# Chemical118/TREW

Hardware: AMD Instinct MI355X
Metric: Gbases/s scanned (short 5 32, 150 bp reads) (higher is better)
Workload: dtype u32

## Files before the change

### trew_amd/csrc/kernels/prefilter.inc

```


#ifdef TREW_MARK_READ_SETUP
#define TREW_SETUP_MARK(n) asm volatile("; MARK " #n)
#else
#define TREW_SETUP_MARK(n)
#endif

__device__ __forceinline__ u32 xor_and(u32 x, u32 y, u32 m) { return __builtin_amdgcn_bitop3_b32(x, y, m, 0x28); }

__device__ __forceinline__ u64 all_k_mask(int kmin, int kmax) {
    if (kmax < kmin) return 0;
    u64 hi = kmax >= 64 ? ~0ull : ((1ull << kmax) - 1ull);
    u64 lo = (1ull << (kmin - 1)) - 1ull;
    return hi & ~lo;
}

template <int NW, int WS>
__device__ __forceinline__ u32 shr_word(const u32 (&x)[NW], int j, u32 bs) {
    const u32 lo = (j + WS < NW) ? x[j + WS < NW ? j + WS : 0] : 0u;
    const u32 hi = (j + WS + 1 < NW) ? x[j + WS + 1 < NW ? j + WS + 1 : 0] : 0u;
    return alignbit(hi, lo, bs);
}

template <int NW, int WS, int NWW>
// ... 346 lines not shown
}
__device__ __forceinline__ u32 halves_note(u32 acc, u32 x, u32 t) { return __builtin_amdgcn_bitop3_b32(acc, x, t, 0x40); }
struct Thr8 {
    int4 a, b;
};
__device__ __forceinline__ Thr8 load_thr8(const int4 *p) {
    typedef int v8i __attribute__((ext_vector_type(8)));
    typedef const __attribute__((address_space(4))) v8i *cptr;
    const v8i v = *(cptr) (unsigned long long) p;
    Thr8 o;
    o.a = make_int4(v[0], v[1], v[2], v[3]);
    o.b = make_int4(v[4], v[5], v[6], v[7]);
    return o;
}
__device__ __forceinline__ int4 load_thr4(const int4 *p) {
    typedef int v4i __attribute__((ext_vector_type(4)));
    typedef const __attribute__((address_space(4))) v4i *cptr;
    const v4i v = *(cptr) (unsigned long long) p;
    return make_int4(v.x, v.y, v.z, v.w);
}

__device__ __forceinline__ const int4 *joint_thresholds(const int2 *thr_tab) { return (const int4 *) (thr_tab + kThrRows * kThrRow); }

__device__ __forceinline__ void filter_halves_uni(const HalvesP &A, const HalvesP &Bh, int L, int klo, int khi, const int4 *__restrict__ thr_row,
                                                  const u32 *wm_tab, bool &passA, bool &passB) {
    u32 accA = 0xffffffffu, accB = 0xffffffffu;
    int k = klo;
    const int4 *tp = thr_row + (klo - 1);
    {
        int b = L - 64;
        b = b > khi ? khi : b;
        auto probe = [&](u32 bs, const int4 t) __attribute__((always_inline)) {
            u32 xA, tA, xB, tB;
            halves_signs(A.P1[0] ^ alignbit(A.P1[1], A.P1[0], bs), A.P2[0] ^ alignbit(A.P2[1], A.P2[0], bs), A.P1[1] ^ alignbit(A.P1[2], A.P1[1], bs),
                         A.P2[1] ^ alignbit(A.P2[2], A.P2[1], bs), t.x, t.y, t.z, xA, tA);
            halves_signs(Bh.P1[0] ^ alignbit(Bh.P1[1], Bh.P1[0], bs), Bh.P2[0] ^ alignbit(Bh.P2[1], Bh.P2[0], bs), Bh.P1[1] ^ alignbit(Bh.P1[2], Bh.P1[1], bs),
                         Bh.P2[1] ^ alignbit(Bh.P2[2], Bh.P2[1], bs), t.x, t.y, t.z, xB, tB);
            accA = halves_note(accA, xA, tA);
            accB = halves_note(accB, xB, tB);
        };
        for (; k + 1 <= b; k += 2, tp += 2) {
            const Thr8 t8 = load_thr8(tp);
            probe((u32) k, t8.a);
            probe((u32) k + 1u, t8.b);
        }
        if (k <= b) {
// ... 51 lines not shown
    V[0] &= alignbit(V[1], V[0], 1u);
    V[1] &= alignbit(V[2], V[1], 1u);
    V[2] &= V[2] >> 1;
}
template <int N>
__device__ __forceinline__ int drain_signs(const u32 (&F1)[N], const u32 (&F2)[N], const int4 th) {
    u32 a = (u32) th.x, b = (u32) th.x, c = (u32) th.y;
#pragma unroll
    for (int j = 0; j < N; j++) {
        a = bcnt_acc(F1[j], a);
        b = bcnt_acc(F2[j], b);
        c = bcnt_acc(F1[j] & F2[j], c);
    }
    const u32 p = a - c, q = b - c;
    const u32 t = a + q + (u32) th.z;
    return (int) __builtin_amdgcn_bitop3_b32(__builtin_amdgcn_bitop3_b32(p, q, c, 0x80), t, t, 0x30);
}
template <int N>
__device__ __forceinline__ bool drain_pass8(const u32 (&F1)[N], const u32 (&F2)[N], const u32 (&F3)[N], const u32 (&V)[N], u32 count, int ithr) {
    const u32 m8 = max_bucket8<N>(F1, F2, F3, V, count);
    return (int) m8 >= ithr;
}

__device__ __forceinline__ bool drain_uni_applies(const DevParams &P, u32 UL, int gmax_run) {
    const int n_halves = P.mode == TREW_MODE_PAIR ? 4 : (P.mode == TREW_MODE_SHORT ? 2 : 0);
    if (n_halves == 0) return false;
    for (int slot = n_halves; slot < mode_slots(P.mode); slot++)
        if (get_segment(P.mode, slot, UL, UL, P.min_mer, P.max_mer, P.slice_len).valid) return false;
    const Segment first = get_segment(P.mode, 0, UL, UL, P.min_mer, P.max_mer, P.slice_len);
    for (int p = 0; p < n_halves; p += 2) {
        const Segment a = get_segment(P.mode, p, UL, UL, P.min_mer, P.max_mer, P.slice_len);
        const Segment b = get_segment(P.mode, p + 1, UL, UL, P.min_mer, P.max_mer, P.slice_len);
        const int la = (int) a.len, lb = (int) b.len, lmin = la < lb ? la : lb, lmax = la < lb ? lb : la;
        const int khi = a.kmax < gmax_run ? a.kmax : gmax_run;
        if (!(a.valid && b.valid && a.kmin == b.kmin && a.kmax == b.kmax && lmax <= 95 && lmax - lmin <= 1 && a.kmin >= 1 && khi <= lmin)) return false;
        if (a.kmin != first.kmin || a.kmax != first.kmax) return false;
    }
    return true;
}

__device__ __forceinline__ u64 drain_probe3(const DrainHalf &h, u32 bs, u64 flag, const int4 *cnt_thr) {
    const u32 cnt = bcnt_acc(h.V[2], bcnt_acc(h.V[1], __popc(h.V[0])));
    const int4 th = cnt_thr[cnt];
    u32 F1[3], F2[3];
#pragma unroll
    for (int j = 0; j < 3; j++) {
        F1[j] = xor_and(h.P1[j], alignbit(j < 2 ? h.P1[j < 2 ? j + 1 : 0] : 0u, h.P1[j], bs), h.V[j]);
        F2[j] = xor_and(h.P2[j], alignbit(j < 2 ? h.P2[j < 2 ? j + 1 : 0] : 0u, h.P2[j], bs), h.V[j]);
    }
    const u64 p4 = __ballot(drain_signs<3>(F1, F2, th) >= 0);
    u64 p8 = 0;
    if (p4 & ~flag) {
        u32 F3[3];
#pragma unroll
        for (int j = 0; j < 3; j++) F3[j] = h.P3[j] ^ alignbit(j < 2 ? h.P3[j < 2 ? j + 1 : 0] : 0u, h.P3[j], bs);
        p8 = __ballot(drain_pass8<3>(F1, F2, F3, h.V, cnt, th.w));
    }
    return p8;
}
__device__ __forceinline__ u64 drain_probe2(const DrainHalf &h, u64 Q1, u64 Q2, u64 V, int s, int k, u64 flag, const int4 *cnt_thr) {
    const u32 v0 = (u32) V, v1 = (u32) (V >> 32);
    const u32 cnt = bcnt_acc(v1, __popc(v0));
    const int4 th = cnt_thr[cnt];
    const u32 sh = (u32) (k - s);
    const u64 S1 = Q1 >> sh, S2 = Q2 >> sh;
    const u32 F1[2] = {xor_and(h.P1[0], (u32) S1, v0), xor_and(h.P1[1], (u32) (S1 >> 32), v1)};
    const u32 F2[2] = {xor_and(h.P2[0], (u32) S2, v0), xor_and(h.P2[1], (u32) (S2 >> 32), v1)};
    const u64 p4 = __ballot(drain_signs<2>(F1, F2, th) >= 0);
    u64 p8 = 0;
    if (p4 & ~flag) {
        const u64 S3 = container64(h.P3, s) >> sh;
        const u32 F3[2] = {h.P3[0] ^ (u32) S3, h.P3[1] ^ (u32) (S3 >> 32)};
        const u32 Vw[2] = {v0, v1};
        p8 = __ballot(drain_pass8<2>(F1, F2, F3, Vw, cnt, th.w));
    }
    return p8;
}

__device__ __forceinline__ bool filter_deferred_uni(const DevParams &P, const DevBatch &B, u64 unit, bool active, int gmax_run,
                                                    const int4 *cnt_thr) {
    const u32 UL = B.uniform_length;
    ReadRef rd[2];
    unit_reads(P, B, unit, active, rd);
    const u64 actm = __ballot(active);
    u64 flag = 0;
    const int n_halves = P.mode == TREW_MODE_PAIR ? 4 : 2;
    for (int p = 0; p < n_halves && flag != actm; p += 2) {
        const Segment sA = get_segment(P.mode, p, UL, UL, P.min_mer, P.max_mer, P.slice_len);
        const Segment sB = get_segment(P.mode, p + 1, UL, UL, P.min_mer, P.max_mer, P.slice_len);
        const int LA = rfl_i((int) sA.len), LB = rfl_i((int) sB.len), Lmax = LA < LB ? LB : LA;
        const int klo = rfl_i(sA.kmin > P.min_mer ? sA.kmin : P.min_mer), khi = rfl_i(sA.kmax < gmax_run ? sA.kmax : gmax_run);
        DrainHalf A, Bh;
        {
            u32 lo[3], hi[3], nm[3];
            load_planes<3>(sA.mate ? rd[1] : rd[0], sA.start, lo, hi, nm);
            drain_half_init(lo, hi, nm, LA, active, A);
            load_planes<3>(sB.mate ? rd[1] : rd[0], sB.start, lo, hi, nm);
            drain_half_init(lo, hi, nm, LB, active, Bh);
        }
        for (int t = 1; t < klo; t++) {
            drain_v_step3(A.V);
            drain_v_step3(Bh.V);
        }
        int k = klo;
        for (const int b = khi < Lmax - 64 ? khi : Lmax - 64; k <= b && flag != actm; k++) {
            flag |= drain_probe3(A, (u32) k, flag, cnt_thr);
            flag |= drain_probe3(Bh, (u32) k, flag, cnt_thr);
            drain_v_step3(A.V);
            drain_v_step3(Bh.V);
        }
        if (k <= khi && flag != actm) {
            const int oA = LA > 63 ? LA - 63 : 0, oB = LB > 63 ? LB - 63 : 0;
            const u64 QA1 = container64(A.P1, oA), QA2 = container64(A.P2, oA), QB1 = container64(Bh.P1, oB), QB2 = container64(Bh.P2, oB);
            u64 VA = ((u64) A.V[1] << 32) | A.V[0], VB = ((u64) Bh.V[1] << 32) | Bh.V[0];
            for (; k <= khi && flag != actm; k++) {
                flag |= drain_probe2(A, QA1, QA2, VA, oA, k, flag, cnt_thr);
                flag |= drain_probe2(Bh, QB1, QB2, VB, oB, k, flag, cnt_thr);
                VA &= VA >> 1;
                VB &= VB >> 1;
            }
        }
    }
    return (flag >> lane_id()) & 1ull;
}

__device__ __forceinline__ bool filter_deferred_half(const DevParams &P, const DevBatch &B, u64 unit, u32 half, bool active, int gmax_run,
                                                     const int4 *cnt_thr) {
    const u32 UL = B.uniform_length;
    ReadRef rd[2];
    unit_reads(P, B, unit, active, rd);
    Segment sg = get_segment(P.mode, 0, UL, UL, P.min_mer, P.max_mer, P.slice_len);
    int Lmax = (int) sg.len;
    const int n_halves = P.mode == TREW_MODE_PAIR ? 4 : 2;
    for (int slot = 1; slot < n_halves; slot++) {
        const Segment o = get_segment(P.mode, slot, UL, UL, P.min_mer, P.max_mer, P.slice_len);
        Lmax = (int) o.len > Lmax ? (int) o.len : Lmax;
        if (half == (u32) slot) {
            sg.mate = o.mate;
            sg.start = o.start;
            sg.len = o.len;
        }
    }
    Lmax = rfl_i(Lmax);
    const int L = (int) sg.len;
    const int klo = rfl_i(sg.kmin > P.min_mer ? sg.kmin : P.min_mer), khi = rfl_i(sg.kmax < gmax_run ? sg.kmax : gmax_run);
    DrainHalf h;
    {
        u32 lo[3], hi[3], nm[3];
        load_planes<3>(sg.mate ? rd[1] : rd[0], sg.start, lo, hi, nm);
        drain_half_init(lo, hi, nm, L, active, h);
    }
    for (int t = 1; t < klo; t++) drain_v_step3(h.V);
    const u64 actm = __ballot(active);
    u64 flag = 0;
    int k = klo;
    for (const int b = khi < Lmax - 64 ? khi : Lmax - 64; k <= b && flag != actm; k++) {
        flag |= drain_probe3(h, (u32) k, flag, cnt_thr);
        drain_v_step3(h.V);
    }
    if (k <= khi && flag != actm) {
        const int o = L > 63 ? L - 63 : 0;
        const u64 Q1 = container64(h.P1, o), Q2 = container64(h.P2, o);
        u64 V = ((u64) h.V[1] << 32) | h.V[0];
        for (; k <= khi && flag != actm; k++) {
            flag |= drain_probe2(h, Q1, Q2, V, o, k, flag, cnt_thr);
            V &= V >> 1;
        }
    }
    return (flag >> lane_id()) & 1ull;
}

constexpr u32 kFilterThreads = TREW_FILTER_THREADS;
// ... 26 lines not shown
            __syncthreads();
            const u32 fb = flush_base;
            for (u32 i = threadIdx.x; i < n; i += blockDim.x) {
                if (fb + i < wl_cap)
                    wl[fb + i] = stage[i];
                else
                    atomicAdd(&diag[kDiagWorklistDrop], 1u);
            }
            __syncthreads();
            if (threadIdx.x == 0) stage_n = 0;
        }
        __syncthreads();
    };
    auto append = [&](bool flag, u32 unit) __attribute__((always_inline)) {
        wave_append(&stage_n, flag, [&](u32 at) __attribute__((always_inline)) { stage[at] = unit; });
        __syncthreads();
        const bool full = stage_n > kStage - kFilterThreads;
        defer_seen = defer_n;
        if constexpr (NW == 3) half_seen = half_n;
        __syncthreads();
        if (full) flush();
    };
    const int nslots = mode_slots(P.mode);
    const int gmax_run = (P.flags & TREW_FLAG_DEBUG_NO_KLOOP) ? P.min_mer - 1 : P.max_mer;
    auto general = [&](u64 unit, bool active) __attribute__((always_inline)) -> u64 {
        ReadRef rd[2];
        unit_reads(P, B, unit, active, rd);
        u64 any = 0;
#pragma unroll
        for (int slot = 0; slot < kMaxSlots; slot++) {
            if (slot < nslots) {
                u64 mask = 0;
                Segment sg = get_segment(P.mode, slot, rd[0].len, rd[1].len, P.min_mer, P.max_mer, P.slice_len);
                const bool ok = active && sg.valid && sg.len <= (u32) (32 * NW - 1);
                if (__any(ok)) {
                    u32 lo[NW], hi[NW], nm[NW];
                    const ReadRef &r = sg.mate ? rd[1] : rd[0];
                    if (ok) {
                        load_planes<NW>(r, sg.start, lo, hi, nm);
                    } else {
#pragma unroll
                        for (int j = 0; j < NW; j++) {
                            lo[j] = hi[j] = 0;
                            nm[j] = 0xffffffffu;
                        }
                    }
                    u64 m;
// ... 1 lines not shown
                        m = all_k_mask(sg.kmin, sg.kmax);
                    else
                        m = filter_segment<NW>(lo, hi, nm, ok ? (int) sg.len : 0, sg.kmin, sg.kmax, P.min_mer, gmax_run, max_seg, P.lowf);
                    mask = ok ? m : 0ull;
                }
                if (active && sg.valid && sg.len > (u32) (32 * NW - 1)) mask = all_k_mask(sg.kmin, sg.kmax);
                any |= mask;
                if (dbg_masks && active && slot < dbg_slots) dbg_masks[unit * (u64) dbg_slots + slot] = mask;
            }
        }
        return any;
    };

    __shared__ u32 defer[kDefer];
    __shared__ unsigned char defer_kind[kDefer];
    constexpr u32 kHalfDefer = NW == 3 ? kDefer : 1;
    __shared__ u32 hdefer[kHalfDefer];
    __shared__ unsigned char hdefer_kind[kHalfDefer];
    __shared__ u32 wm_tab[34];
    if (threadIdx.x < 34) wm_tab[threadIdx.x] = threadIdx.x < 32 ? 0xffffffffu >> threadIdx.x : 0u;
    __shared__ int4 cnt_thr[kCntThr];
    for (u32 i = threadIdx.x; i < (u32) kCntThr; i += blockDim.x) cnt_thr[i] = count_thresholds((int) i, P.lowf);
    const u32 UL = B.uniform_length;
    const bool uni = NW <= 5 && UL != 0 && thr_tab != nullptr && P.mode != TREW_MODE_LONG && !(P.flags & TREW_FLAG_NO_FILTER);
    const bool uni_drain = NW == 3 && uni && !dbg_masks && !(P.flags & TREW_FLAG_DEBUG_NO_UNI_DRAIN) && drain_uni_applies(P, UL, gmax_run);
    if (threadIdx.x == 0) defer_n = 0;
    if constexpr (NW == 3) {
        if (threadIdx.x == 0) half_n = 0;
    }
    __syncthreads();
    __shared__ u32 next_chunk[2];
    constexpr u32 kChunkShards = 8;
    const u32 my_shard = blockIdx.x & (kChunkShards - 1u);
    auto shard_ctr = [&](u32 sh) __attribute__((always_inline)) { return wl_count + 32u + 32u * sh + kChunkCounterWord; };
    u64 chunk = blockIdx.x;
    u32 round = 0;
    for (;;) {
        const bool more = chunk * kFilterThreads < B.n_units;
        if (more) {
            const u64 unit = chunk * kFilterThreads + threadIdx.x;
            const bool active = unit < B.n_units;
            u32 nxt = 0;
            if (threadIdx.x == 0) nxt = gridDim.x + kChunkShards * atomicAdd(shard_ctr(my_shard), 1u) + my_shard;
            u64 any = 0;
            bool dfr = active, dfr_n = false;
            bool dfr_half = false;
            u32 hsel = 0;
            if constexpr (NW <= 5) {
                if (uni) {
                    TREW_SETUP_MARK(read_setup);
                    ReadRef rd[2];
                    unit_reads(P, B, unit, active, rd);
                    dfr = false;
                    int slot0 = 0;
                    if constexpr (NW == 3) {
                        const int n_halves = P.mode == TREW_MODE_PAIR ? 4 : (P.mode == TREW_MODE_SHORT ? 2 : 0);
                        u32 nneed = 0;
                        for (; slot0 + 1 < n_halves && !dbg_masks && !(P.flags & TREW_FLAG_DEBUG_NO_JOINT); slot0 += 2) {
                            const Segment sA = get_segment(P.mode, slot0, UL, UL, P.min_mer, P.max_mer, P.slice_len);
                            const Segment sB = get_segment(P.mode, slot0 + 1, UL, UL, P.min_mer, P.max_mer, P.slice_len);
                            const int L = rfl_i((int) sA.len);
                            const int klo = rfl_i(sA.kmin > P.min_mer ? sA.kmin : P.min_mer), khi = rfl_i(sA.kmax < gmax_run ? sA.kmax : gmax_run);
                            const bool uneq = sB.len == sA.len + 1u;
                            if (!(sA.valid && sB.valid && (sA.len == sB.len || uneq) && sA.len <= 95u && sA.kmin == sB.kmin && sA.kmax == sB.kmax &&
                                  klo >= L + 1 - kUniSubsetMax && khi <= L - 32 && klo <= 31))
                                break;
                            HalvesP hp, hq;
                            u32 np, nq;
                            u32 slot_p = (u32) slot0, slot_q = (u32) slot0 + 1u;
                            const bool a_left = sA.start == 0u;
                            const u32 h = rfl(a_left ? sB.start : sA.start), len_l = rfl(a_left ? sA.len : sB.len), len_r = rfl(a_left ? sB.len : sA.len);
                            const bool one_load = UL <= 159u && sA.mate == sB.mate && (a_left ? sA.start : sB.start) == 0u && (h >> 5) == 2u && h + len_r <= UL;
                            if (one_load) {
                                TREW_SETUP_MARK(one_load);
                                ReadPlanes5 r;
                                load_read5(sA.mate ? rd[1] : rd[0], r);
                                np = read5_left_has_n(r.nm, (int) len_l);
                                nq = read5_right_has_n(r.nm, (int) h, (int) len_r);
                                if (!a_left) slot_p = (u32) slot0 + 1u, slot_q = (u32) slot0;
#ifndef TREW_AB_NO_READ_PREFIX
                                halves_prefix_read5(r, h & 31u, hp, hq);
#else
                                u32 loq[3], hiq[3];
                                read5_from64(r.lo, h & 31u, loq);
                                read5_from64(r.hi, h & 31u, hiq);
                                const u32 lop[3] = {r.lo[0], r.lo[1], r.lo[2]}, hip[3] = {r.hi[0], r.hi[1], r.hi[2]};
                                halves_prefix(lop, hip, L, hp);
                                halves_prefix(loq, hiq, L, hq);
#endif
                            } else {
                                TREW_SETUP_MARK(two_loads);
                                u32 loA[3], hiA[3], nmA[3], loB[3], hiB[3], nmB[3];
                                load_planes<3>(sA.mate ? rd[1] : rd[0], sA.start, loA, hiA, nmA);
                                load_planes<3>(sB.mate ? rd[1] : rd[0], sB.start, loB, hiB, nmB);
                                np = segment_has_n<3>(nmA, L), nq = segment_has_n<3>(nmB, (int) sB.len);
                                halves_prefix(loA, hiA, L, hp);
                                halves_prefix(loB, hiB, L, hq);
                            }
                            dfr_n = dfr_n || (active && (np | nq) != 0);
                            bool passp, passq;
                            TREW_SETUP_MARK(joint_loop);
                            filter_halves_uni(hp, hq, L, klo, khi, joint_thresholds(thr_tab) + (uneq ? 2 + slot0 / 2 : slot0 / 2) * kThrRow, wm_tab, passp, passq);
                            const bool needp = active && (np != 0 || passp), needq = active && (nq != 0 || passq);
                            nneed += (u32) needp + (u32) needq;
                            hsel = needq ? slot_q : (needp ? slot_p : hsel);
                            dfr = dfr || needp || needq;
                        }
                        dfr_half = uni_drain && slot0 == n_halves && nneed == 1u;
                    }
                    for (int slot = slot0; slot < nslots; slot++) {
                        const Segment sg = get_segment(P.mode, slot, UL, UL, P.min_mer, P.max_mer, P.slice_len);
                        if (!sg.valid) continue;
                        if (sg.len > (u32) (32 * NW - 1)) {
                            dfr = dfr || active;
                            continue;
                        }
                        u32 lo[NW], hi[NW], nm[NW];
                        const ReadRef r = sg.mate ? rd[1] : rd[0];
                        load_planes<NW>(r, sg.start, lo, hi, nm);
                        u32 anyn = 0;
#pragma unroll
                        for (int j = 0; j < NW; j++) {
                            const int bits = (int) sg.len - 32 * j;
                            const u32 lm = low_mask(bits);
                            anyn |= nm[j] & lm;
                        }
                        UniVerdict vd;
                        filter_segment_uni<NW>(lo, hi, (int) sg.len, sg.kmin, sg.kmax, P.min_mer, gmax_run, thr_tab + slot * kThrRow, dbg_masks != nullptr, vd);
                        dfr = dfr || (active && anyn != 0);
                        dfr_n = dfr_n || (active && anyn != 0);
                        any |= (vd.flagm >> lane_id()) & 1ull;
                        if (dbg_masks && active && anyn == 0 && slot < dbg_slots)
                            dbg_masks[unit * (u64) dbg_slots + slot] = ((((u64) vd.chi) << 32) | vd.clo) & all_k_mask(sg.kmin, sg.kmax);
                    }
                }
            }
            {
                wave_append(&defer_n, dfr && !dfr_half, [=](u32 at) __attribute__((always_inline)) {
                    defer[at] = (u32) unit;
                    defer_kind[at] = dfr_n ? 1 : 0;
                });
                if constexpr (NW == 3) wave_append(&half_n, dfr_half, [=](u32 at) __attribute__((always_inline)) {
                    hdefer[at] = (u32) unit;
                    hdefer_kind[at] = (unsigned char) ((hsel << 1) | (dfr_n ? 1u : 0u));
                });
            }
            if (threadIdx.x == 0) next_chunk[round & 1u] = nxt;
            append(active && !dfr && any != 0, (u32) unit);
            chunk = next_chunk[round & 1u];
            if (chunk * kFilterThreads >= B.n_units) {
                __syncthreads();
                if (threadIdx.x == 0) {
                    u64 c = chunk;
                    for (u32 att = 1; att < kChunkShards && c * kFilterThreads >= B.n_units; att++) {
                        const u32 sh = (my_shard + att) & (kChunkShards - 1u);
                        c = (u64) gridDim.x + (u64) kChunkShards * atomicAdd(shard_ctr(sh), 1u) + sh;
                    }
                    next_chunk[round & 1u] = (u32) (c < 0xffffffffull ? c : 0xffffffffull);
                }
                __syncthreads();
                chunk = next_chunk[round & 1u];
                __syncthreads();
            }
            round++;
        }
        const u32 dn = defer_seen, hn = half_seen;
        auto drain = [&](const u32 *list, const unsigned char *kind, u32 *list_n, u32 n, bool halves) __attribute__((always_inline)) {
            const u32 take = n < kFilterThreads ? n : kFilterThreads;
            const u32 at = n - take;
            const bool active2 = threadIdx.x < take;
            const u32 unit2 = active2 ? list[at + threadIdx.x] : 0u;
            const u32 kind2 = active2 ? kind[at + threadIdx.x] : 0u;
            const bool n2 = (kind2 & 1u) != 0;
            __syncthreads();
            if (threadIdx.x == 0) {
                *list_n = at;
                if (halves || uni_drain) atomicAdd(&g_fallback[halves ? kFallbackHalfDrain : kFallbackUnitDrain], take);
            }
#if !defined(TREW_AB_SKIP_DRAIN) && !defined(TREW_AB_SKIP_UNIT_DRAIN)
            const u64 any2 = halves      ? (u64) filter_deferred_half(P, B, unit2, kind2 >> 1, active2, gmax_run, cnt_thr)
                             : uni_drain ? (u64) filter_deferred_uni(P, B, unit2, active2, gmax_run, cnt_thr)
                                         : general(unit2, active2);
#else
#ifdef TREW_AB_SKIP_DRAIN
            constexpr bool kSkipHalves = true;
#else
            constexpr bool kSkipHalves = false;
#endif
            u64 any2 = 0;
            if (halves && !kSkipHalves) {
                any2 = (u64) filter_deferred_half(P, B, unit2, kind2 >> 1, active2, gmax_run, cnt_thr);
            } else {
                u32 keep = unit2 + kind2;
                asm volatile("" : "+v"(keep), "+v"(any2));
                (void) keep;
            }
#endif
            append(active2 && any2 != 0 && !n2, unit2);
            append(active2 && any2 != 0 && n2, unit2);
        };
        const bool drain_units = dn >= kFilterThreads || (!more && dn > 0u), drain_halves = NW == 3 && (hn >= kFilterThreads || (!more && hn > 0u));
        if (drain_units || drain_halves) {
            if (drain_units) drain(defer, defer_kind, &defer_n, dn, false);
            if constexpr (NW == 3) {
                if (drain_halves) drain(hdefer, hdefer_kind, &half_n, hn, true);
            }
        } else if (!more) {
            break;
        }
    }
    flush();
}
```

### trew_amd/csrc/trew_capi.cpp

```cpp
#include <hip/hip_runtime.h>

#include <algorithm>
#include <atomic>
#include <cmath>
#include <cstdio>
#include <cstdlib>
#include <cstring>
#include <mutex>
#include <string>
#include <thread>
#include <vector>

#include "trew_common.hpp"
#include "trew_launch.hpp"
#include "trew_measures_host.hpp"
#include "trew_synth.hpp"

using namespace trew;

namespace {

enum Measure { kAnnotate, kTracts, kIntervals, kVariants, kPeriods, kChain, kRepeats, kSatellites, kAlign, kRefine, kTandems, kTrace, kDecompose, kDissect, kResolve, kMonomers, kCopies, kMeasures };
const char *const kMeasureName[kMeasures] = {"annotate", "tracts", "intervals", "variants", "periods", "chain", "repeats", "satellites", "align", "refine", "tandems", "trace", "decompose", "dissect", "resolve", "monomers", "copies"};
const bool kMeasureHasMotifs[kMeasures] = {true, true, true, true, false, true, false, false, true, false, false, true, false, false, false, false, false};
// ... 14 lines not shown
    int n_motifs = 0;
    u32 k[kAnnotMaxMotifs] = {};
    DevBuf rows;
    DevBuf aligned;
    u64 max_rows = 0;
};

struct Slot {
    hipStream_t stream = nullptr;
    u32 *d_buf = nullptr;
    u32 *d_words = nullptr, *d_offsets = nullptr, *d_lengths = nullptr;
    unsigned char *d_ascii = nullptr;
    u32 *d_wl = nullptr;
    u32 *d_wl_count = nullptr;
    u32 *d_bnd = nullptr;
    u32 bnd_cap = 0;
    u32 *d_live = nullptr;
    bool live_launch = false;
    int2 *d_thr = nullptr;
    int2 *h_thr = nullptr;
    hipEvent_t ev_tail = nullptr, ev_copied = nullptr;
    u32 *h_seen = nullptr;
    u32 thr_length = 0;
    SegResults res = {nullptr, nullptr, nullptr, nullptr};
    static constexpr int kRing = 128;
    hipEvent_t ev[kRing][3] = {};
    u64 n_launches = 0;
    u64 n_submits = 0;
    u64 n_reported = 0;
    u64 n_units = 0;
    AnnotMotifDev *d_motifs = nullptr, *h_motifs = nullptr;
    int motifs_staged = 0;
    trew_hip_monomer *d_monomers = nullptr, *h_monomers = nullptr;
    int monomers_staged = 0;
    MeasureState measure[kMeasures];
};

thread_local std::string g_init_error;
thread_local std::string g_thread_error;
constexpr size_t kWlCountWords = 32 + 8 * 32;
constexpr size_t kWlCountBytes = kWlCountWords * 4;

}

struct trew_hip_ctx {
    trew_hip_params p;
// ... 449 lines not shown
            db->words = s.d_buf;
            db->offsets = s.d_buf + b->n_words;
            db->lengths = s.d_buf + b->n_words + b->n_reads;
            return 0;
        }
        if (int rc = bc.copy(s.d_words, b->words, b->n_words * 4)) return rc;
        db->words = s.d_words;
        db->offsets = nullptr;
        db->lengths = nullptr;
        if (b->offsets) {
            if (int rc = bc.copy(s.d_offsets, b->offsets, b->n_reads * 4)) return rc;
            if (int rc = bc.copy(s.d_lengths, b->lengths, b->n_reads * 4)) return rc;
            db->offsets = s.d_offsets;
            db->lengths = s.d_lengths;
        }
        if (int rc = bc.end()) return rc;
    }
    return 0;
}

static int stage_thresholds(trew_hip_ctx *ctx, Slot &s, const DevBatch &db, const int2 **out) {
    *out = nullptr;
    if (db.offsets || db.lengths || db.uniform_length == 0) return 0;
    if (s.thr_length != db.uniform_length) {
        HIPCHK(ctx, hipStreamSynchronize(s.stream));
        fill_thresholds(ctx->dp, db.uniform_length, s.h_thr);
        HIPCHK(ctx, hipMemcpyAsync(s.d_thr, s.h_thr, kThrTableBytes, hipMemcpyHostToDevice, s.stream));
        s.thr_length = db.uniform_length;
    }
    *out = s.d_thr;
    return 0;
}

static int sync_all(trew_hip_ctx *ctx);

static int launch_batch(trew_hip_ctx *ctx, Slot &s, const DevBatch &db, u32 max_seg, u32 max_len) {
    s.n_units = db.n_units;
    if (db.n_units == 0) return 0;
    if (ctx->p.mode == TREW_MODE_SEGMENT) {
        HIPCHK(ctx, hipMemsetAsync(s.res.k_high, 0, db.n_reads * 4, s.stream));
        HIPCHK(ctx, hipMemsetAsync(s.res.k_low, 0, db.n_reads * 4, s.stream));
        HIPCHK(ctx, hipMemsetAsync(s.res.seq_high, 0, db.n_reads * 8, s.stream));
        HIPCHK(ctx, hipMemsetAsync(s.res.seq_low, 0, db.n_reads * 8, s.stream));
        HIPCHK(ctx, hipMemsetAsync(s.res.seq_high_hi, 0, db.n_reads * 8, s.stream));
        HIPCHK(ctx, hipMemsetAsync(s.res.seq_low_hi, 0, db.n_reads * 8, s.stream));
    }
    const u32 wl_cap = (u32) ctx->p.max_batch_reads;
    u32 *const wl_count = s.d_wl_count + (s.n_launches & 1) * kWlCountWords;
    u32 *const wl_count_next = s.d_wl_count + ((s.n_launches + 1) & 1) * kWlCountWords;
    auto submit_failed = [&](int rc) {
        const std::string keep = g_thread_error;
// ... 1674 lines not shown
```

### trew_amd/csrc/trew_common.hpp

```cpp
#pragma once
#include <stdint.h>

#include "../../include/trew_hip.h"

namespace trew {

typedef uint32_t u32;
typedef uint64_t u64;

constexpr int kMaxSlots = 6;
constexpr int kMaxSegBases = 1023;
constexpr int kTablePartBits = 9;
constexpr int kThrRows = kMaxSlots + 2;
constexpr int kThrJointRows = 4;
constexpr int kThrRow = 66;
constexpr size_t kThrTableBytes = (size_t) kThrRows * kThrRow * 8 + (size_t) kThrJointRows * kThrRow * 16;
constexpr int kThrNever = 1 << 20;

struct DevParams {
    int min_mer, max_mer;
    double low, high;
    float lowf;
    int slice_len;
    int mode;
    u32 flags;
};

struct DevBatch {
    const u32 *words;
    const u32 *offsets;
    const u32 *lengths;
    u32 uniform_length;
    u32 uniform_stride;
    u64 n_reads;
    u64 n_units;
};

constexpr int kChunkCounterWord = 16;
constexpr int kStoredPrefixWord = 1;
// ... 197 lines not shown
        }
        s.valid = true;
    } else {
        if (slot != 0 || n1 == 0) return s;
        s.kmin = MIN_MER;
        s.kmax = MAX_MER;
        s.start = 0;
        s.len = n1;
        s.valid = true;
    }
    return s;
}

constexpr int kUniSubsetMax = 72;
TREW_HD inline int uni_windows(int nw, int L, int k) {
    const int W = L - k + 1;
    return (nw == 3 && W > 64 && W <= kUniSubsetMax) ? 64 : W;
}

TREW_HD inline int mode_slots(int mode) {
    return mode == TREW_MODE_SHORT ? 3 : mode == TREW_MODE_PAIR ? 6 : mode == TREW_MODE_LONG ? 2 : 1;
}

}
```

### trew_amd/csrc/trew_kernels.hip

```cpp
#include <hip/hip_runtime.h>

#include <algorithm>
#include <cstdlib>

#include "trew_common.hpp"
#include "trew_launch.hpp"
#include "trew_synth.hpp"

#ifndef TREW_FILTER_THREADS
#define TREW_FILTER_THREADS 256
#endif

namespace trew {

typedef unsigned __int128 u128;

#include "kernels/helpers.inc"
#include "kernels/bound.inc"
#include "kernels/prefilter.inc"
#include "kernels/count_table.inc"
#include "kernels/exact_core.inc"
#include "kernels/decide_group.inc"
#include "kernels/bounds_pass.inc"
#include "kernels/driver_long.inc"
// ... 61 lines not shown
        for (int k = 1; k <= kThrRow; k++) {
            int2 th;
            th.x = kThrNever;
            th.y = -1;
            const int WA = (int) a.len - k + 1, WB = WA + 1;
            if (ok && WA > 0) {
                const int Weff = uni_windows(nw, (int) a.len, k);
                const volatile float pa = (float) WA * P.lowf, pb = (float) WB * P.lowf;
                const int xa = (int) floorf(pa) + 1 - (WA - Weff), xb = (int) floorf(pb) + 1 - (WB - Weff);
                th.x = std::min(xa, xb);
                th.y = Weff - th.x;
            }
            table[(kMaxSlots + p) * kThrRow + k - 1] = th;
        }
    }
    int4 *joint = (int4 *) (table + kThrRows * kThrRow);
    for (int r = 0; r < kThrJointRows; r++) {
        const int2 *src = table + (r < 2 ? 2 * r : kMaxSlots + (r - 2)) * kThrRow;
        for (int k = 1; k <= kThrRow; k++) {
            const int2 th = src[k - 1];
            joint[r * kThrRow + k - 1] = make_int4(-2 * th.x, -th.x, 3 * th.x - th.y - 1, th.x);
        }
    }
}

hipError_t launch_filter(hipStream_t st, u32 n_cu, u32 max_seg_len, const DevParams &P, const DevBatch &B, u32 *wl, u32 *wl_count,
                         u32 wl_cap, u64 *dbg_masks, int dbg_slots, u32 *diag, const int2 *d_thr) {
    const int nw = pick_nw(max_seg_len);
    const int max_seg = (int) std::min<u32>(max_seg_len, (u32) (32 * nw - 1));
    if (B.n_units == 0) return hipSuccess;
    typedef void (*kern_t)(DevParams, DevBatch, u32 *, u32 *, u32, u64 *, int, int, u32 *, const int2 *);
    const kern_t fn = nw == 3 ? filter_kernel<3> : nw == 5 ? filter_kernel<5> : nw == 10 ? filter_kernel<10> : filter_kernel<32>;
    const u32 threads = kFilterThreads;
    static thread_local kern_t cached_fn = nullptr;
    static thread_local int cached_per_cu = 0;
    int per_cu = cached_per_cu;
    if (cached_fn != fn) {
        if (hipOccupancyMaxActiveBlocksPerMultiprocessor(&per_cu, (const void *) fn, (int) threads, 0) != hipSuccess || per_cu < 1) per_cu = 4;
        if (const char *e = getenv("TREW_FILTER_BLOCKS_PER_CU")) per_cu = std::max(1, atoi(e));
        cached_fn = fn;
        cached_per_cu = per_cu;
    }
    u64 blocks = (B.n_units + threads - 1) / threads;
    const u64 persistent = (u64) n_cu * (u64) per_cu;
    if (blocks > persistent) blocks = persistent;
    hipLaunchKernelGGL(fn, dim3((u32) blocks), dim3(threads), 0, st, P, B, wl, wl_count, wl_cap, dbg_masks, dbg_slots, max_seg, diag, d_thr);
// ... 286 lines not shown
```

Before: 2200.

## Precompute per-batch filter segment geometry on host and load it via scalar loads

```diff
diff --git a/trew_amd/csrc/kernels/prefilter.inc b/trew_amd/csrc/kernels/prefilter.inc
--- a/trew_amd/csrc/kernels/prefilter.inc
+++ b/trew_amd/csrc/kernels/prefilter.inc
@@ -392,6 +392,45 @@
 
 __device__ __forceinline__ const int4 *joint_thresholds(const int2 *thr_tab) { return (const int4 *) (thr_tab + kThrRows * kThrRow); }
 
+__device__ __forceinline__ const FilterGeom *filter_geom(const int2 *thr_tab, bool masks) {
+    return (const FilterGeom *) ((const char *) thr_tab + kThrGeomOffset) + (masks ? 1 : 0);
+}
+template <typename T>
+__device__ __forceinline__ T load_geom(const T *p) {
+    constexpr int N = (int) (sizeof(T) / 4);
+    static_assert(N == 8 || N == 16, "one scalar load");
+    typedef u32 vNu __attribute__((ext_vector_type(N)));
+    typedef const __attribute__((address_space(4))) vNu *cptr;
+    const vNu v = *(cptr) p;
+    T o;
+    __builtin_memcpy(&o, &v, sizeof(T));
+    return o;
+}
+__device__ __forceinline__ const FilterGeom *geom_here(const FilterGeom *g, u32 tick) {
+    asm("" : "+s"(g) : "s"(tick));
+    return g;
+}
+__device__ __forceinline__ ReadRef uniform_read(const DevBatch &B, u32 reads_per_unit, u64 unit, u32 mate, bool active, u32 read_words) {
+    ReadRef r;
+    r.w = B.words + (active ? (unit * reads_per_unit + mate) * (u64) B.uniform_stride : 0ull);
+    r.len = active ? B.uniform_length : 0u;
+    r.nw = active ? read_words : 0u;
+    return r;
+}
+__device__ __forceinline__ ReadRef uniform_read(const DevBatch &B, u32 reads_per_unit, u64 unit, u32 mate, bool active) {
+    return uniform_read(B, reads_per_unit, unit, mate, active, (B.uniform_length + 31u) >> 5);
+}
+__device__ __forceinline__ void halves_prefix_masked(const u32 (&lo)[3], const u32 (&hi)[3], const u32 (&lm)[3], HalvesP &o) {
+    u32 f1[3], f2[3];
+#pragma unroll
+    for (int j = 0; j < 3; j++) {
+        f1[j] = lo[j] & lm[j];
+        f2[j] = hi[j] & lm[j];
+    }
+    prefix_parity<3>(f1, o.P1);
+    prefix_parity<3>(f2, o.P2);
+}
+
 __device__ __forceinline__ void filter_halves_uni(const HalvesP &A, const HalvesP &Bh, int L, int klo, int khi, const int4 *__restrict__ thr_row,
                                                   const u32 *wm_tab, bool &passA, bool &passB) {
     u32 accA = 0xffffffffu, accB = 0xffffffffu;
@@ -489,23 +528,6 @@
     return (int) m8 >= ithr;
 }
 
-__device__ __forceinline__ bool drain_uni_applies(const DevParams &P, u32 UL, int gmax_run) {
-    const int n_halves = P.mode == TREW_MODE_PAIR ? 4 : (P.mode == TREW_MODE_SHORT ? 2 : 0);
-    if (n_halves == 0) return false;
-    for (int slot = n_halves; slot < mode_slots(P.mode); slot++)
-        if (get_segment(P.mode, slot, UL, UL, P.min_mer, P.max_mer, P.slice_len).valid) return false;
-    const Segment first = get_segment(P.mode, 0, UL, UL, P.min_mer, P.max_mer, P.slice_len);
-    for (int p = 0; p < n_halves; p += 2) {
-        const Segment a = get_segment(P.mode, p, UL, UL, P.min_mer, P.max_mer, P.slice_len);
-        const Segment b = get_segment(P.mode, p + 1, UL, UL, P.min_mer, P.max_mer, P.slice_len);
-        const int la = (int) a.len, lb = (int) b.len, lmin = la < lb ? la : lb, lmax = la < lb ? lb : la;
-        const int khi = a.kmax < gmax_run ? a.kmax : gmax_run;
-        if (!(a.valid && b.valid && a.kmin == b.kmin && a.kmax == b.kmax && lmax <= 95 && lmax - lmin <= 1 && a.kmin >= 1 && khi <= lmin)) return false;
-        if (a.kmin != first.kmin || a.kmax != first.kmax) return false;
-    }
-    return true;
-}
-
 __device__ __forceinline__ u64 drain_probe3(const DrainHalf &h, u32 bs, u64 flag, const int4 *cnt_thr) {
     const u32 cnt = bcnt_acc(h.V[2], bcnt_acc(h.V[1], __popc(h.V[0])));
     const int4 th = cnt_thr[cnt];
@@ -544,25 +566,24 @@
     return p8;
 }
 
-__device__ __forceinline__ bool filter_deferred_uni(const DevParams &P, const DevBatch &B, u64 unit, bool active, int gmax_run,
+__device__ __forceinline__ bool filter_deferred_uni(const DevParams &P, const DevBatch &B, u64 unit, bool active, const FilterGeom *geom, u32 tick,
                                                     const int4 *cnt_thr) {
-    const u32 UL = B.uniform_length;
-    ReadRef rd[2];
-    unit_reads(P, B, unit, active, rd);
+    const FilterGeom *g = geom_here(geom, tick);
+    const GeomHead hd = load_geom(&g->head);
+    const u32 rpu = P.mode == TREW_MODE_PAIR ? 2u : 1u;
     const u64 actm = __ballot(active);
     u64 flag = 0;
-    const int n_halves = P.mode == TREW_MODE_PAIR ? 4 : 2;
+    const int n_halves = (int) hd.n_halves;
     for (int p = 0; p < n_halves && flag != actm; p += 2) {
-        const Segment sA = get_segment(P.mode, p, UL, UL, P.min_mer, P.max_mer, P.slice_len);
-        const Segment sB = get_segment(P.mode, p + 1, UL, UL, P.min_mer, P.max_mer, P.slice_len);
-        const int LA = rfl_i((int) sA.len), LB = rfl_i((int) sB.len), Lmax = LA < LB ? LB : LA;
-        const int klo = rfl_i(sA.kmin > P.min_mer ? sA.kmin : P.min_mer), khi = rfl_i(sA.kmax < gmax_run ? sA.kmax : gmax_run);
+        const SlotGeom sA = load_geom(&g->slot[p]), sB = load_geom(&g->slot[p + 1]);
+        const int LA = (int) sA.len, LB = (int) sB.len, Lmax = LA < LB ? LB : LA;
+        const int klo = hd.drain_klo, khi = hd.drain_khi;
         DrainHalf A, Bh;
         {
             u32 lo[3], hi[3], nm[3];
-            load_planes<3>(sA.mate ? rd[1] : rd[0], sA.start, lo, hi, nm);
+            load_planes<3>(uniform_read(B, rpu, unit, sA.mate, active), sA.start, lo, hi, nm);
             drain_half_init(lo, hi, nm, LA, active, A);
-            load_planes<3>(sB.mate ? rd[1] : rd[0], sB.start, lo, hi, nm);
+            load_planes<3>(uniform_read(B, rpu, unit, sB.mate, active), sB.start, lo, hi, nm);
             drain_half_init(lo, hi, nm, LB, active, Bh);
         }
         for (int t = 1; t < klo; t++) {
@@ -591,30 +612,19 @@
     return (flag >> lane_id()) & 1ull;
 }
 
-__device__ __forceinline__ bool filter_deferred_half(const DevParams &P, const DevBatch &B, u64 unit, u32 half, bool active, int gmax_run,
+__device__ __forceinline__ bool filter_deferred_half(const DevParams &P, const DevBatch &B, u64 unit, u32 half, bool active, const FilterGeom *geom, u32 tick,
                                                      const int4 *cnt_thr) {
-    const u32 UL = B.uniform_length;
-    ReadRef rd[2];
-    unit_reads(P, B, unit, active, rd);
-    Segment sg = get_segment(P.mode, 0, UL, UL, P.min_mer, P.max_mer, P.slice_len);
-    int Lmax = (int) sg.len;
-    const int n_halves = P.mode == TREW_MODE_PAIR ? 4 : 2;
-    for (int slot = 1; slot < n_halves; slot++) {
-        const Segment o = get_segment(P.mode, slot, UL, UL, P.min_mer, P.max_mer, P.slice_len);
-        Lmax = (int) o.len > Lmax ? (int) o.len : Lmax;
-        if (half == (u32) slot) {
-            sg.mate = o.mate;
-            sg.start = o.start;
-            sg.len = o.len;
-        }
-    }
-    Lmax = rfl_i(Lmax);
-    const int L = (int) sg.len;
-    const int klo = rfl_i(sg.kmin > P.min_mer ? sg.kmin : P.min_mer), khi = rfl_i(sg.kmax < gmax_run ? sg.kmax : gmax_run);
+    const FilterGeom *g = geom_here(geom, tick);
+    const GeomHead hd = load_geom(&g->head);
+    const u32 rpu = P.mode == TREW_MODE_PAIR ? 2u : 1u;
+    const SlotGeom *mine = &g->slot[half < hd.n_halves ? half : 0u];
+    const u32 mate = mine->mate, start = mine->start;
+    const int L = (int) mine->len;
+    const int Lmax = hd.drain_lmax, klo = hd.drain_klo, khi = hd.drain_khi;
     DrainHalf h;
     {
         u32 lo[3], hi[3], nm[3];
-        load_planes<3>(sg.mate ? rd[1] : rd[0], sg.start, lo, hi, nm);
+        load_planes<3>(uniform_read(B, rpu, unit, mate, active), start, lo, hi, nm);
         drain_half_init(lo, hi, nm, L, active, h);
     }
     for (int t = 1; t < klo; t++) drain_v_step3(h.V);
@@ -687,7 +697,7 @@
         if (full) flush();
     };
     const int nslots = mode_slots(P.mode);
-    const int gmax_run = (P.flags & TREW_FLAG_DEBUG_NO_KLOOP) ? P.min_mer - 1 : P.max_mer;
+    const int gmax_run = filter_gmax_run(P);
     auto general = [&](u64 unit, bool active) __attribute__((always_inline)) -> u64 {
         ReadRef rd[2];
         unit_reads(P, B, unit, active, rd);
@@ -735,8 +745,22 @@
     __shared__ int4 cnt_thr[kCntThr];
     for (u32 i = threadIdx.x; i < (u32) kCntThr; i += blockDim.x) cnt_thr[i] = count_thresholds((int) i, P.lowf);
     const u32 UL = B.uniform_length;
-    const bool uni = NW <= 5 && UL != 0 && thr_tab != nullptr && P.mode != TREW_MODE_LONG && !(P.flags & TREW_FLAG_NO_FILTER);
-    const bool uni_drain = NW == 3 && uni && !dbg_masks && !(P.flags & TREW_FLAG_DEBUG_NO_UNI_DRAIN) && drain_uni_applies(P, UL, gmax_run);
+    const FilterGeom *geom = thr_tab ? filter_geom(thr_tab, dbg_masks != nullptr) : nullptr;
+    const bool uni = NW <= 5 && UL != 0 && thr_tab != nullptr && P.mode != TREW_MODE_LONG && !(P.flags & TREW_FLAG_NO_FILTER) &&
+                     load_geom(&geom->head).nw == (u32) NW;
+    const bool uni_drain = NW == 3 && uni && !dbg_masks && !(P.flags & TREW_FLAG_DEBUG_NO_UNI_DRAIN) && load_geom(&geom->head).drain_ok != 0u;
+#ifdef TREW_AB_PIN_GEOM
+    GeomHead hd_pin = {};
+    HalvesRound hr_pin = {};
+    if (uni) {
+        hd_pin = load_geom(&geom->head);
+        hr_pin = load_geom(&geom->round[0]);
+    }
+    asm volatile("" : "+s"(hd_pin.n_halves), "+s"(hd_pin.n_joint), "+s"(hd_pin.n_slots));
+    asm volatile("" : "+s"(hr_pin.L), "+s"(hr_pin.klo), "+s"(hr_pin.khi), "+s"(hr_pin.row), "+s"(hr_pin.one_load), "+s"(hr_pin.mate), "+s"(hr_pin.bs),
+                 "+s"(hr_pin.slot_p), "+s"(hr_pin.slot_q), "+s"(hr_pin.read_words));
+    asm volatile("" : "+s"(hr_pin.nl[0]), "+s"(hr_pin.nl[1]), "+s"(hr_pin.nl[2]), "+s"(hr_pin.nr[0]), "+s"(hr_pin.nr[1]), "+s"(hr_pin.nr[2]));
+#endif
     if (threadIdx.x == 0) defer_n = 0;
     if constexpr (NW == 3) {
         if (threadIdx.x == 0) half_n = 0;
@@ -762,75 +786,73 @@
             if constexpr (NW <= 5) {
                 if (uni) {
                     TREW_SETUP_MARK(read_setup);
-                    ReadRef rd[2];
-                    unit_reads(P, B, unit, active, rd);
+                    const FilterGeom *g = geom_here(geom, round);
+#ifndef TREW_AB_PIN_GEOM
+                    const GeomHead hd = load_geom(&g->head);
+#else
+                    const GeomHead hd = hd_pin;
+#endif
+                    const u32 rpu = P.mode == TREW_MODE_PAIR ? 2u : 1u;
                     dfr = false;
-                    int slot0 = 0;
+                    u32 first = 0;
                     if constexpr (NW == 3) {
-                        const int n_halves = P.mode == TREW_MODE_PAIR ? 4 : (P.mode == TREW_MODE_SHORT ? 2 : 0);
+                        const u32 n_joint = hd.n_joint;
                         u32 nneed = 0;
-                        for (; slot0 + 1 < n_halves && !dbg_masks && !(P.flags & TREW_FLAG_DEBUG_NO_JOINT); slot0 += 2) {
-                            const Segment sA = get_segment(P.mode, slot0, UL, UL, P.min_mer, P.max_mer, P.slice_len);
-                            const Segment sB = get_segment(P.mode, slot0 + 1, UL, UL, P.min_mer, P.max_mer, P.slice_len);
-                            const int L = rfl_i((int) sA.len);
-                            const int klo = rfl_i(sA.kmin > P.min_mer ? sA.kmin : P.min_mer), khi = rfl_i(sA.kmax < gmax_run ? sA.kmax : gmax_run);
-                            const bool uneq = sB.len == sA.len + 1u;
-                            if (!(sA.valid && sB.valid && (sA.len == sB.len || uneq) && sA.len <= 95u && sA.kmin == sB.kmin && sA.kmax == sB.kmax &&
-                                  klo >= L + 1 - kUniSubsetMax && khi <= L - 32 && klo <= 31))
-                                break;
+                        for (u32 pr = 0; pr < n_joint; pr++) {
+#ifndef TREW_AB_PIN_GEOM
+                            const HalvesRound hr = load_geom(&g->round[pr]);
+#else
+                            const HalvesRound hr = hr_pin;
+#endif
                             HalvesP hp, hq;
                             u32 np, nq;
-                            u32 slot_p = (u32) slot0, slot_q = (u32) slot0 + 1u;
-                            const bool a_left = sA.start == 0u;
-                            const u32 h = rfl(a_left ? sB.start : sA.start), len_l = rfl(a_left ? sA.len : sB.len), len_r = rfl(a_left ? sB.len : sA.len);
-                            const bool one_load = UL <= 159u && sA.mate == sB.mate && (a_left ? sA.start : sB.start) == 0u && (h >> 5) == 2u && h + len_r <= UL;
-                            if (one_load) {
+                            if (hr.one_load) {
                                 TREW_SETUP_MARK(one_load);
                                 ReadPlanes5 r;
-                                load_read5(sA.mate ? rd[1] : rd[0], r);
-                                np = read5_left_has_n(r.nm, (int) len_l);
-                                nq = read5_right_has_n(r.nm, (int) h, (int) len_r);
-                                if (!a_left) slot_p = (u32) slot0 + 1u, slot_q = (u32) slot0;
+                                load_read5(uniform_read(B, rpu, unit, hr.mate, active, hr.read_words), r);
+                                np = (r.nm[0] & hr.nl[0]) | (r.nm[1] & hr.nl[1]) | (r.nm[2] & hr.nl[2]);
+                                nq = (r.nm[2] & hr.nr[0]) | (r.nm[3] & hr.nr[1]) | (r.nm[4] & hr.nr[2]);
 #ifndef TREW_AB_NO_READ_PREFIX
-                                halves_prefix_read5(r, h & 31u, hp, hq);
+                                halves_prefix_read5(r, hr.bs, hp, hq);
 #else
                                 u32 loq[3], hiq[3];
-                                read5_from64(r.lo, h & 31u, loq);
-                                read5_from64(r.hi, h & 31u, hiq);
+                                read5_from64(r.lo, hr.bs, loq);
+                                read5_from64(r.hi, hr.bs, hiq);
                                 const u32 lop[3] = {r.lo[0], r.lo[1], r.lo[2]}, hip[3] = {r.hi[0], r.hi[1], r.hi[2]};
-                                halves_prefix(lop, hip, L, hp);
-                                halves_prefix(loq, hiq, L, hq);
+                                halves_prefix(lop, hip, hr.L, hp);
+                                halves_prefix(loq, hiq, hr.L, hq);
 #endif
                             } else {
                                 TREW_SETUP_MARK(two_loads);
+                                const HalvesLoads hl = load_geom(&g->loads[pr]);
                                 u32 loA[3], hiA[3], nmA[3], loB[3], hiB[3], nmB[3];
-                                load_planes<3>(sA.mate ? rd[1] : rd[0], sA.start, loA, hiA, nmA);
-                                load_planes<3>(sB.mate ? rd[1] : rd[0], sB.start, loB, hiB, nmB);
-                                np = segment_has_n<3>(nmA, L), nq = segment_has_n<3>(nmB, (int) sB.len);
-                                halves_prefix(loA, hiA, L, hp);
-                                halves_prefix(loB, hiB, L, hq);
+                                load_planes<3>(uniform_read(B, rpu, unit, hl.mate_a, active, hr.read_words), hl.start_a, loA, hiA, nmA);
+                                load_planes<3>(uniform_read(B, rpu, unit, hl.mate_b, active, hr.read_words), hl.start_b, loB, hiB, nmB);
+                                np = (nmA[0] & hr.nl[0]) | (nmA[1] & hr.nl[1]) | (nmA[2] & hr.nl[2]);
+                                nq = (nmB[0] & hr.nr[0]) | (nmB[1] & hr.nr[1]) | (nmB[2] & hr.nr[2]);
+                                halves_prefix_masked(loA, hiA, hr.nl, hp);
+                                halves_prefix_masked(loB, hiB, hr.nl, hq);
                             }
                             dfr_n = dfr_n || (active && (np | nq) != 0);
                             bool passp, passq;
                             TREW_SETUP_MARK(joint_loop);
-                            filter_halves_uni(hp, hq, L, klo, khi, joint_thresholds(thr_tab) + (uneq ? 2 + slot0 / 2 : slot0 / 2) * kThrRow, wm_tab, passp, passq);
+                            filter_halves_uni(hp, hq, hr.L, hr.klo, hr.khi, joint_thresholds(thr_tab) + hr.row * (u32) kThrRow, wm_tab, passp, passq);
                             const bool needp = active && (np != 0 || passp), needq = active && (nq != 0 || passq);
                             nneed += (u32) needp + (u32) needq;
-                            hsel = needq ? slot_q : (needp ? slot_p : hsel);
+                            hsel = needq ? hr.slot_q : (needp ? hr.slot_p : hsel);
                             dfr = dfr || needp || needq;
                         }
-                        dfr_half = uni_drain && slot0 == n_halves && nneed == 1u;
+                        first = 2u * n_joint;
+                        dfr_half = uni_drain && first == hd.n_halves && nneed == 1u;
                     }
-                    for (int slot = slot0; slot < nslots; slot++) {
-                        const Segment sg = get_segment(P.mode, slot, UL, UL, P.min_mer, P.max_mer, P.slice_len);
-                        if (!sg.valid) continue;
-                        if (sg.len > (u32) (32 * NW - 1)) {
+                    for (u32 i = first; i < hd.n_slots; i++) {
+                        const SlotGeom sg = load_geom(&g->slot[i < (u32) kMaxSlots ? i : 0u]);
+                        if (sg.too_long) {
                             dfr = dfr || active;
                             continue;
                         }
                         u32 lo[NW], hi[NW], nm[NW];
-                        const ReadRef r = sg.mate ? rd[1] : rd[0];
-                        load_planes<NW>(r, sg.start, lo, hi, nm);
+                        load_planes<NW>(uniform_read(B, rpu, unit, sg.mate, active), sg.start, lo, hi, nm);
                         u32 anyn = 0;
 #pragma unroll
                         for (int j = 0; j < NW; j++) {
@@ -839,12 +861,12 @@
                             anyn |= nm[j] & lm;
                         }
                         UniVerdict vd;
-                        filter_segment_uni<NW>(lo, hi, (int) sg.len, sg.kmin, sg.kmax, P.min_mer, gmax_run, thr_tab + slot * kThrRow, dbg_masks != nullptr, vd);
+                        filter_segment_uni<NW>(lo, hi, (int) sg.len, sg.kmin, sg.kmax, P.min_mer, gmax_run, thr_tab + sg.slot * (u32) kThrRow, dbg_masks != nullptr, vd);
                         dfr = dfr || (active && anyn != 0);
                         dfr_n = dfr_n || (active && anyn != 0);
                         any |= (vd.flagm >> lane_id()) & 1ull;
-                        if (dbg_masks && active && anyn == 0 && slot < dbg_slots)
-                            dbg_masks[unit * (u64) dbg_slots + slot] = ((((u64) vd.chi) << 32) | vd.clo) & all_k_mask(sg.kmin, sg.kmax);
+                        if (dbg_masks && active && anyn == 0 && (int) sg.slot < dbg_slots)
+                            dbg_masks[unit * (u64) dbg_slots + sg.slot] = ((((u64) vd.chi) << 32) | vd.clo) & all_k_mask(sg.kmin, sg.kmax);
                     }
                 }
             }
@@ -891,8 +913,8 @@
                 if (halves || uni_drain) atomicAdd(&g_fallback[halves ? kFallbackHalfDrain : kFallbackUnitDrain], take);
             }
 #if !defined(TREW_AB_SKIP_DRAIN) && !defined(TREW_AB_SKIP_UNIT_DRAIN)
-            const u64 any2 = halves      ? (u64) filter_deferred_half(P, B, unit2, kind2 >> 1, active2, gmax_run, cnt_thr)
-                             : uni_drain ? (u64) filter_deferred_uni(P, B, unit2, active2, gmax_run, cnt_thr)
+            const u64 any2 = halves      ? (u64) filter_deferred_half(P, B, unit2, kind2 >> 1, active2, geom, round, cnt_thr)
+                             : uni_drain ? (u64) filter_deferred_uni(P, B, unit2, active2, geom, round, cnt_thr)
                                          : general(unit2, active2);
 #else
 #ifdef TREW_AB_SKIP_DRAIN
@@ -902,7 +924,7 @@
 #endif
             u64 any2 = 0;
             if (halves && !kSkipHalves) {
-                any2 = (u64) filter_deferred_half(P, B, unit2, kind2 >> 1, active2, gmax_run, cnt_thr);
+                any2 = (u64) filter_deferred_half(P, B, unit2, kind2 >> 1, active2, geom, round, cnt_thr);
             } else {
                 u32 keep = unit2 + kind2;
                 asm volatile("" : "+v"(keep), "+v"(any2));
diff --git a/trew_amd/csrc/trew_capi.cpp b/trew_amd/csrc/trew_capi.cpp
--- a/trew_amd/csrc/trew_capi.cpp
+++ b/trew_amd/csrc/trew_capi.cpp
@@ -60,6 +60,7 @@
     hipEvent_t ev_tail = nullptr, ev_copied = nullptr;
     u32 *h_seen = nullptr;
     u32 thr_length = 0;
+    u32 thr_flags = 0;
     SegResults res = {nullptr, nullptr, nullptr, nullptr};
     static constexpr int kRing = 128;
     hipEvent_t ev[kRing][3] = {};
@@ -555,11 +556,12 @@
 static int stage_thresholds(trew_hip_ctx *ctx, Slot &s, const DevBatch &db, const int2 **out) {
     *out = nullptr;
     if (db.offsets || db.lengths || db.uniform_length == 0) return 0;
-    if (s.thr_length != db.uniform_length) {
+    if (s.thr_length != db.uniform_length || s.thr_flags != ctx->dp.flags) {
         HIPCHK(ctx, hipStreamSynchronize(s.stream));
         fill_thresholds(ctx->dp, db.uniform_length, s.h_thr);
         HIPCHK(ctx, hipMemcpyAsync(s.d_thr, s.h_thr, kThrTableBytes, hipMemcpyHostToDevice, s.stream));
         s.thr_length = db.uniform_length;
+        s.thr_flags = ctx->dp.flags;
     }
     *out = s.d_thr;
     return 0;
diff --git a/trew_amd/csrc/trew_common.hpp b/trew_amd/csrc/trew_common.hpp
--- a/trew_amd/csrc/trew_common.hpp
+++ b/trew_amd/csrc/trew_common.hpp
@@ -14,7 +14,6 @@
 constexpr int kThrRows = kMaxSlots + 2;
 constexpr int kThrJointRows = 4;
 constexpr int kThrRow = 66;
-constexpr size_t kThrTableBytes = (size_t) kThrRows * kThrRow * 8 + (size_t) kThrJointRows * kThrRow * 16;
 constexpr int kThrNever = 1 << 20;
 
 struct DevParams {
@@ -258,4 +257,146 @@
     return mode == TREW_MODE_SHORT ? 3 : mode == TREW_MODE_PAIR ? 6 : mode == TREW_MODE_LONG ? 2 : 1;
 }
 
-}
+
+TREW_HD inline int filter_gmax_run(const DevParams &P) { return (P.flags & TREW_FLAG_DEBUG_NO_KLOOP) ? P.min_mer - 1 : P.max_mer; }
+TREW_HD inline u32 geom_low_mask(int bits) { return bits >= 32 ? 0xffffffffu : (bits <= 0 ? 0u : ((1u << bits) - 1u)); }
+
+TREW_HD inline bool joint_loop_admits(const Segment &a, const Segment &b, int klo, int khi) {
+    const int L = (int) a.len;
+    const bool uneq = b.len == a.len + 1u;
+    return a.valid && b.valid && (a.len == b.len || uneq) && a.len <= 95u && a.kmin == b.kmin && a.kmax == b.kmax &&
+           klo >= L + 1 - kUniSubsetMax && khi <= L - 32 && klo <= 31;
+}
+
+TREW_HD inline bool drain_uni_applies(const DevParams &P, u32 UL, int gmax_run) {
+    const int n_halves = P.mode == TREW_MODE_PAIR ? 4 : (P.mode == TREW_MODE_SHORT ? 2 : 0);
+    if (n_halves == 0) return false;
+    for (int slot = n_halves; slot < mode_slots(P.mode); slot++)
+        if (get_segment(P.mode, slot, UL, UL, P.min_mer, P.max_mer, P.slice_len).valid) return false;
+    const Segment first = get_segment(P.mode, 0, UL, UL, P.min_mer, P.max_mer, P.slice_len);
+    for (int p = 0; p < n_halves; p += 2) {
+        const Segment a = get_segment(P.mode, p, UL, UL, P.min_mer, P.max_mer, P.slice_len);
+        const Segment b = get_segment(P.mode, p + 1, UL, UL, P.min_mer, P.max_mer, P.slice_len);
+        const int la = (int) a.len, lb = (int) b.len, lmin = la < lb ? la : lb, lmax = la < lb ? lb : la;
+        const int khi = a.kmax < gmax_run ? a.kmax : gmax_run;
+        if (!(a.valid && b.valid && a.kmin == b.kmin && a.kmax == b.kmax && lmax <= 95 && lmax - lmin <= 1 && a.kmin >= 1 && khi <= lmin)) return false;
+        if (a.kmin != first.kmin || a.kmax != first.kmax) return false;
+    }
+    return true;
+}
+
+struct HalvesRound {
+    int L, klo, khi;
+    u32 row;
+    u32 one_load;
+    u32 mate;
+    u32 bs;
+    u32 slot_p, slot_q;
+    u32 nl[3], nr[3];
+    u32 read_words;
+};
+struct HalvesLoads {
+    u32 mate_a, start_a, mate_b, start_b;
+    u32 pad[4];
+};
+struct SlotGeom {
+    u32 slot, mate, start, len;
+    int kmin, kmax;
+    u32 too_long, pad;
+};
+struct GeomHead {
+    u32 nw;
+    u32 n_halves;
+    u32 n_joint;
+    u32 n_slots;
+    u32 drain_ok;
+    int drain_klo, drain_khi;
+    int drain_lmax;
+};
+struct FilterGeom {
+    HalvesRound round[2];
+    HalvesLoads loads[2];
+    SlotGeom slot[kMaxSlots];
+    GeomHead head;
+    u32 pad[8];
+};
+static_assert(sizeof(HalvesRound) == 64 && sizeof(HalvesLoads) == 32 && sizeof(SlotGeom) == 32 && sizeof(GeomHead) == 32, "one scalar load each");
+constexpr size_t kThrGeomOffset = (size_t) kThrRows * kThrRow * 8 + (size_t) kThrJointRows * kThrRow * 16;
+static_assert(kThrGeomOffset % 64 == 0 && sizeof(FilterGeom) % 64 == 0, "the block's lines are aligned");
+constexpr size_t kThrTableBytes = kThrGeomOffset + 2 * sizeof(FilterGeom);
+
+TREW_HD inline void build_filter_geom(const DevParams &P, u32 UL, int nw, FilterGeom *g) {
+    const int gmax_run = filter_gmax_run(P);
+    const int nslots = mode_slots(P.mode);
+    GeomHead &hd = g->head;
+    hd.nw = (u32) nw;
+    hd.n_halves = P.mode == TREW_MODE_PAIR ? 4u : (P.mode == TREW_MODE_SHORT ? 2u : 0u);
+    hd.n_joint = 0;
+    hd.n_slots = 0;
+    for (int j = 0; j < 8; j++) g->pad[j] = 0;
+    for (int i = 0; i < kMaxSlots; i++) {
+        SlotGeom &o = g->slot[i];
+        o.slot = o.mate = o.start = o.len = 0;
+        o.kmin = 1, o.kmax = 0;
+        o.too_long = o.pad = 0;
+    }
+    for (int slot = 0; slot < nslots; slot++) {
+        const Segment sg = get_segment(P.mode, slot, UL, UL, P.min_mer, P.max_mer, P.slice_len);
+        if (!sg.valid) continue;
+        SlotGeom &o = g->slot[hd.n_slots++];
+        o.slot = (u32) slot, o.mate = sg.mate, o.start = sg.start, o.len = sg.len;
+        o.kmin = sg.kmin, o.kmax = sg.kmax;
+        o.too_long = sg.len > (u32) (32 * nw - 1) ? 1u : 0u;
+    }
+    bool joint = nw == 3 && !(P.flags & TREW_FLAG_DEBUG_NO_JOINT);
+    for (int p = 0; p < 2; p++) {
+        HalvesRound &r = g->round[p];
+        HalvesLoads &l = g->loads[p];
+        r.L = r.klo = 0, r.khi = -1;
+        r.row = r.one_load = r.mate = r.bs = r.slot_p = r.slot_q = 0;
+        r.read_words = (UL + 31u) >> 5;
+        for (int j = 0; j < 3; j++) r.nl[j] = r.nr[j] = 0;
+        l.mate_a = l.start_a = l.mate_b = l.start_b = 0;
+        for (int j = 0; j < 4; j++) l.pad[j] = 0;
+        if (2 * p + 1 >= (int) hd.n_halves) joint = false;
+        if (!joint) continue;
+        const Segment a = get_segment(P.mode, 2 * p, UL, UL, P.min_mer, P.max_mer, P.slice_len);
+        const Segment b = get_segment(P.mode, 2 * p + 1, UL, UL, P.min_mer, P.max_mer, P.slice_len);
+        const int klo = a.kmin > P.min_mer ? a.kmin : P.min_mer, khi = a.kmax < gmax_run ? a.kmax : gmax_run;
+        if (!joint_loop_admits(a, b, klo, khi)) {
+            joint = false;
+            continue;
+        }
+        hd.n_joint = (u32) p + 1u;
+        r.L = (int) a.len, r.klo = klo, r.khi = khi;
+        const bool uneq = b.len == a.len + 1u;
+        r.row = (u32) (uneq ? 2 + p : p);
+        l.mate_a = a.mate, l.start_a = a.start, l.mate_b = b.mate, l.start_b = b.start;
+        const bool a_left = a.start == 0u;
+        const u32 h = a_left ? b.start : a.start, len_l = a_left ? a.len : b.len, len_r = a_left ? b.len : a.len;
+        r.one_load = (UL <= 159u && a.mate == b.mate && (a_left ? a.start : b.start) == 0u && (h >> 5) == 2u && h + len_r <= UL) ? 1u : 0u;
+        r.mate = a.mate;
+        r.bs = h & 31u;
+        r.slot_p = (u32) (2 * p), r.slot_q = (u32) (2 * p + 1);
+        if (r.one_load) {
+            if (!a_left) r.slot_p = (u32) (2 * p + 1), r.slot_q = (u32) (2 * p);
+            for (int j = 0; j < 3; j++) {
+                r.nl[j] = geom_low_mask((int) len_l - 32 * j);
+                r.nr[j] = geom_low_mask((int) (h + len_r) - 32 * (j + 2)) & ~geom_low_mask((int) h - 32 * (j + 2));
+            }
+        } else {
+            for (int j = 0; j < 3; j++) {
+                r.nl[j] = geom_low_mask(r.L - 32 * j);
+                r.nr[j] = geom_low_mask((int) b.len - 32 * j);
+            }
+        }
+    }
+    hd.drain_ok = drain_uni_applies(P, UL, gmax_run) ? 1u : 0u;
+    const Segment first = get_segment(P.mode, 0, UL, UL, P.min_mer, P.max_mer, P.slice_len);
+    hd.drain_klo = first.kmin > P.min_mer ? first.kmin : P.min_mer;
+    hd.drain_khi = first.kmax < gmax_run ? first.kmax : gmax_run;
+    hd.drain_lmax = 0;
+    for (u32 i = 0; i < hd.n_halves && i < hd.n_slots; i++) hd.drain_lmax = (int) g->slot[i].len > hd.drain_lmax ? (int) g->slot[i].len : hd.drain_lmax;
+}
+
+}
diff --git a/trew_amd/csrc/trew_kernels.hip b/trew_amd/csrc/trew_kernels.hip
--- a/trew_amd/csrc/trew_kernels.hip
+++ b/trew_amd/csrc/trew_kernels.hip
@@ -107,6 +107,11 @@
             joint[r * kThrRow + k - 1] = make_int4(-2 * th.x, -th.x, 3 * th.x - th.y - 1, th.x);
         }
     }
+    FilterGeom *geom = (FilterGeom *) ((char *) table + kThrGeomOffset);
+    build_filter_geom(P, uniform_length, nw, &geom[0]);
+    DevParams no_joint = P;
+    no_joint.flags |= TREW_FLAG_DEBUG_NO_JOINT;
+    build_filter_geom(no_joint, uniform_length, nw, &geom[1]);
 }
 
 hipError_t launch_filter(hipStream_t st, u32 n_cu, u32 max_seg_len, const DevParams &P, const DevBatch &B, u32 *wl, u32 *wl_count,
```

Result: faster. 2273 (median of 6 runs) (+3.3%).
